# TIGER-AI-Lab/AnyV2V

Measured on AMD Instinct MI355X. Metric: frames/sec for 16fx512x512 DDIM-inversion+PnP-edit; spatial-attn MFMA % of peak, higher is better.
Workload: dtype f16; 1 GPU; BASELINE config 3 per GPU: 1 clip x 16f x 512x512, 50-step DDIM inversion (UNet B=1) + 50-step PnP edit (UNet B=3, cfg 9.0, conv+spatial+temporal injection on every step); a bench step = 1 inversion step + 1 edit step = 1/50 clip; I2VGen-XL 3D-UNet 1.42B params, random init; frames=16, hip_graphs=True, finite=True

## Files before the change

anyv2v_amd/_lib.py:

```python
from __future__ import annotations

import ctypes as C
import os

_HERE = os.path.dirname(os.path.abspath(__file__))
LIB_PATH = os.path.join(_HERE, "libanyv2v_hip.so")
ABI_VERSION = 105


class HipExtensionMissing(RuntimeError):
    pass


class HipKernelError(RuntimeError):
    pass


class GemmDesc(C.Structure):
    _fields_ = [
        ("A0", C.c_void_p), ("A1", C.c_void_p), ("W", C.c_void_p), ("C", C.c_void_p),
        ("bias", C.c_void_p), ("rowvec", C.c_void_p), ("R", C.c_void_p),
        ("M", C.c_int32), ("N", C.c_int32), ("C0", C.c_int32), ("C1", C.c_int32),
        ("lda0", C.c_int32), ("lda1", C.c_int32), ("ldc", C.c_int32), ("ldr", C.c_int32),
        ("ldrv", C.c_int32), ("rowvec_div", C.c_int32), ("mode", C.c_int32),
        ("Hi", C.c_int32), ("Wi", C.c_int32), ("Ho", C.c_int32), ("Wo", C.c_int32),
        ("stride", C.c_int32), ("up", C.c_int32), ("asym", C.c_int32), ("F", C.c_int32), ("HW", C.c_int32),
        ("act", C.c_int32), ("flags", C.c_int32),
        ("workspace", C.c_void_p), ("workspace_bytes", C.c_int64),
        ("ln_c1", C.c_void_p), ("ln_eps", C.c_float), ("reserved0", C.c_int32),
        ("gn_stats", C.c_void_p), ("gn_stats_floats", C.c_int64), ("gn_rows_per_group", C.c_int32), ("gn_groups", C.c_int32),
    ]

ANYV2V_GEMM_NAIVE = 1 << 0
ANYV2V_GEMM_LDS_DMA = 1 << 1
ANYV2V_GEMM_NO_BIG = 1 << 2
ANYV2V_GEMM_FORCE_BIG = 1 << 3
ANYV2V_GEMM_NO_SPLITK = 1 << 4
ANYV2V_GEMM_PROBE_TRACE = 1 << 5
ANYV2V_GEMM_PROBE_KO_SHIFT = 6
ANYV2V_GEMM_NO_WS = 1 << 9
ANYV2V_GEMM_FORCE_WS = 1 << 10
ANYV2V_GEMM_NF4 = 1 << 11
ANYV2V_GEMM_NF5 = 1 << 12
ANYV2V_GEMM_RASTER_SHIFT = 13
ANYV2V_GEMM_RASTER_NFAST = 1 << 16
ANYV2V_GEMM_PP = 1 << 17
ANYV2V_GEMM_NO_PP = 1 << 18
ANYV2V_GEMM_PP_192 = 1 << 19
ANYV2V_GEMM_PP_256 = 1 << 20
ANYV2V_GEMM_SW = 1 << 21
ANYV2V_GEMM_NO_SW = 1 << 22
ANYV2V_GEMM_PROBE_SW_KO_SHIFT = 23
ANYV2V_GEMM_STREAMK = 1 << 26
ANYV2V_GEMM_FORCE_STREAMK = 1 << 27
ANYV2V_GEMM_SWH = 1 << 28
ANYV2V_GEMM_PROBE_KORDER_SHIFT = 29


class FFDesc(C.Structure):
    _fields_ = [
        ("X", C.c_void_p), ("W1", C.c_void_p), ("b1", C.c_void_p), ("W2", C.c_void_p), ("b2", C.c_void_p), ("R", C.c_void_p),
        ("Y", C.c_void_p), ("M", C.c_int32), ("C", C.c_int32), ("H", C.c_int32), ("ldx", C.c_int32), ("ldr", C.c_int32),
        ("ldy", C.c_int32), ("flags", C.c_int32), ("reserved0", C.c_int32),
    ]


class AttnDesc(C.Structure):
    _fields_ = [
        ("Q", C.c_void_p), ("K", C.c_void_p), ("V", C.c_void_p), ("O", C.c_void_p),
        ("ldq", C.c_int32), ("ldk", C.c_int32), ("ldv", C.c_int32), ("ldo", C.c_int32),
        ("batch", C.c_int32), ("heads", C.c_int32), ("Sq", C.c_int32), ("Sk", C.c_int32),
        ("inner", C.c_int32),
        ("q_outer", C.c_int64), ("q_inner", C.c_int64), ("q_seq", C.c_int64),
        ("kv_outer", C.c_int64), ("kv_inner", C.c_int64), ("kv_seq", C.c_int64),
        ("kv_div", C.c_int32), ("qk_mod", C.c_int32), ("scale", C.c_float), ("flags", C.c_int32),
    ]


_VP, _I32, _I64, _F32 = C.c_void_p, C.c_int32, C.c_int64, C.c_float
SYMBOLS = {
    "anyv2v_gemm_f16": (C.c_int, [C.POINTER(GemmDesc), _VP]),
    "anyv2v_gemm_gn_stats_floats": (C.c_int64, [C.POINTER(GemmDesc)]),
    "anyv2v_gemm_gn_launches": (C.c_int64, [_I32]),
    "anyv2v_ff_geglu_f16": (C.c_int, [C.POINTER(FFDesc), _VP]),
    "anyv2v_groupnorm_f16": (C.c_int, [_VP, _VP, _I32, _I32, _VP, _VP, _VP, _VP, _I32, _I32, _I32, _F32, _I32, _VP]),
    "anyv2v_groupnorm_scratch_floats": (C.c_int64, [_I32, _I32, _I32]),
    "anyv2v_groupnorm_stats_floats": (C.c_int64, [_I32, _I32, _I32]),
    "anyv2v_groupnorm_apply_stats_f16": (C.c_int, [_VP, _VP, _VP, _VP, _VP, C.POINTER(C.c_int32), _F32, _I32, _VP]),
    "anyv2v_groupnorm_partial_floats": (C.c_int64, [_I32, _I32, _I32, _I32]),
    "anyv2v_groupnorm_partial_f16": (C.c_int, [_VP, _VP, _I32, _I32, _VP, _I32, _I32, _I32, _VP]),
    "anyv2v_groupnorm_apply_f16": (C.c_int, [_VP, _VP, _I32, _I32, _VP, _VP, _VP, _VP, _I32, _I32, _I32, _F32, _I32, _I32, _VP]),
    "anyv2v_groupnorm_pivot_f16": (C.c_int, [_VP, _VP, _I32, _I32, _VP, _I32, _I32, _I32, _I32, _VP]),
    "anyv2v_groupnorm_partial_pivot_f16": (C.c_int, [_VP, _VP, _I32, _I32, _VP, _VP, _I32, _I32, _I32, _VP]),
    "anyv2v_groupnorm_apply_pivot_f16": (C.c_int, [_VP, _VP, _I32, _I32, _VP, _VP, _VP, _VP, _VP, _I32, _I32, _I32, _F32, _I32, _I32, _VP]),
    "anyv2v_layernorm_f16": (C.c_int, [_VP, _VP, _VP, _VP, _I32, _I32, _F32, _VP]),
    "anyv2v_attention_f16": (C.c_int, [C.POINTER(AttnDesc), _VP]),
    "anyv2v_attention_small_f16": (C.c_int, [C.POINTER(AttnDesc), _I32, _VP]),
    "anyv2v_attention_bias_f16": (C.c_int, [C.POINTER(AttnDesc), _I32, _VP, _VP]),
    "anyv2v_softmax_rows_f32_f16": (C.c_int, [_VP, _I32, _VP, _I32, _I32, _I32, _F32, _VP]),
    "anyv2v_silu_f16": (C.c_int, [_VP, _VP, _I64, _VP]),
    "anyv2v_add_f16": (C.c_int, [_VP, _VP, _VP, _I64, _VP]),
    "anyv2v_timestep_embedding_f16": (C.c_int, [_VP, _VP, _I32, _I32, _VP]),
    "anyv2v_ncfhw_to_tokens_f16": (C.c_int, [_VP, _VP, _I32, _I32, _I32, _I32, _I32, _I32, _VP]),
    "anyv2v_tokens_to_ncfhw_f16": (C.c_int, [_VP, _VP, _I32, _I32, _I32, _I32, _I32, _I32, _VP]),
    "anyv2v_adaptive_avgpool_f16": (C.c_int, [_VP, _VP, _I32, _I32, _I32, _I32, _I32, _I32, _VP]),
    "anyv2v_copy_cols_f16": (C.c_int, [_VP, _I32, _I32, _VP, _I32, _I32, _I64, _I32, _VP]),
    "anyv2v_gather_rows_f16": (C.c_int, [_VP, _I32, _I32, _VP, _VP, _I32, _I32, _I64, _I32, _VP]),
    "anyv2v_freeu_f16": (C.c_int, [_VP, _I32, _VP, _I32, _I32, _F32, _VP, _I32, _VP, _I32, _I32, _F32, _I32, _I32, _I32, _VP]),
    "anyv2v_tile_blend_f16": (C.c_int, [_VP, _I64, _I32, _I32, _VP, _VP, _VP, _VP, _I32, _I32, _VP, _I32, _I32, _I32, _VP]),
    "anyv2v_rotary_f16":(C.c_int, [_VP, _I32, _I64, _I32, _I32, _I32, _I32, _I32, _I32, C.c_float, _VP]),
    "anyv2v_cfg_ddim_step_f16": (C.c_int, [_VP, _I32, _I32, _I32, _F32, _VP, _VP, _VP, _I32, _I32, _I32, _VP]),
    "anyv2v_ddim_step_f16": (C.c_int, [_VP, _VP, _VP, _F32, _F32, _F32, _F32, _I64, _VP]),
    "anyv2v_guided_step_f16": (C.c_int, [_VP, _I64, _I32, _I32, _I32, _F32, _F32, _I32, _F32, _F32, _F32, _F32, _VP, _VP, _VP]),
    "anyv2v_guided_step_noise_f16": (C.c_int, [_VP, _I64, _I32, _I32, _I32, _F32, _F32, _I32, _F32, _F32, _F32, _F32, _VP, _VP, _VP, _F32, _VP]),
    "anyv2v_set_batch_hint": (C.c_int, [_I32, _I32]),
    "anyv2v_last_error": (C.c_char_p, []),
    "anyv2v_version": (C.c_int, []),
    "anyv2v_selftest": (C.c_int, [_VP, _I64, _VP]),
}

_lib = None


def load():
    global _lib
    if _lib is not None:
        return _lib
    if not os.path.isfile(LIB_PATH):
        raise HipExtensionMissing(
            f"{LIB_PATH} not found: the HIP kernels are the product path and there is no fallback. "
            f"Build with `make -C {os.path.join(_HERE, 'csrc')}` (or `python -c 'import __graft_entry__ as g; g.build()'`).")
    lib = C.CDLL(LIB_PATH)
    for name, (res, args) in SYMBOLS.items():
        fn = getattr(lib, name)
        fn.restype = res
        fn.argtypes = args
    if lib.anyv2v_version() < ABI_VERSION:
        raise HipExtensionMissing(f"{LIB_PATH} is ABI {lib.anyv2v_version()}, this binding needs >= {ABI_VERSION}: rebuild it "
                                  f"(`make -C {os.path.join(_HERE, 'csrc')}`)")
    _lib = lib
    return lib


def check(rc: int, what: str = ""):
    if rc != 0:
        msg = load().anyv2v_last_error()
        raise HipKernelError(f"{what} failed (rc={rc}): {msg.decode() if msg else ''}")
```

anyv2v_amd/ops.py:

```python
from __future__ import annotations

import ctypes as C
import os
from typing import Optional

import torch

from . import _lib
from ._lib import AttnDesc, GemmDesc

MODE_LINEAR, MODE_CONV2D, MODE_TEMPORAL = 0, 1, 2
ACT_NONE, ACT_SILU, ACT_GELU, ACT_GEGLU, ACT_F32OUT = 0, 1, 2, 3, 4

FORCE_NAIVE = False
ATTN_FLAGS = int(os.environ.get("ANYV2V_ATTN_FLAGS", "0"))
GEMM_FLAGS = int(os.environ.get("ANYV2V_GEMM_FLAGS", "0"))
USE_GLDS = os.environ.get("ANYV2V_GLDS", "1") == "1"


def _parse_switch(value: Optional[str]) -> bool:
    return (value or "0").strip() == "1"


GN_EPILOGUE = _parse_switch(os.environ.get("ANYV2V_GN_EPILOGUE"))
# ... 92 lines not shown
               | GEMM_FLAGS)
    if ln is not None:
        c1, eps = ln
        assert c1.dtype == torch.float32 and c1.is_cuda and c1.numel() >= N and c1.is_contiguous()
        d.ln_c1, d.ln_eps = _p(c1), float(eps)
    ws = _workspace(a0.device)
    d.workspace, d.workspace_bytes = ws.data_ptr(), ws.numel() * 4
    if gn is not None:
        stats, rows_per_group, groups = gn
        d.gn_rows_per_group, d.gn_groups = int(rows_per_group), int(groups)
        if stats is not None:
            assert stats.dtype == torch.float32 and stats.is_cuda and stats.is_contiguous()
            d.gn_stats, d.gn_stats_floats = stats.data_ptr(), stats.numel()
    if _query:
        return int(lib.anyv2v_gemm_gn_stats_floats(C.byref(d)))
    _lib.check(lib.anyv2v_gemm_f16(C.byref(d), _stream()), "anyv2v_gemm_f16")
    return out


def gemm_gn_stats_floats(a0: torch.Tensor, w: torch.Tensor, *, rows_per_group: int, groups: int = 32, **kw) -> int:
    return gemm(a0, w, gn=(None, rows_per_group, groups), _query=True, **kw)


def gn_launches(reset: bool = True) -> int:
    return int(_lib.load().anyv2v_gemm_gn_launches(int(reset)))


def gn_stats_floats(M: int, rows_per_group: int, groups: int = 32) -> int:
    return int(_lib.load().anyv2v_groupnorm_stats_floats(int(M), int(rows_per_group), int(groups)))


def groupnorm_from_stats(x: torch.Tensor, gamma, beta, stats: torch.Tensor, rows_per_group: int, *, groups: int = 32,
                         eps: float = 1e-5, silu: bool = False, out=None):
    lib = _lib.load()
    _rowmajor(x, "X")
    assert x.is_contiguous()
    M, Cc = x.shape
    if out is None:
        out = torch.empty((M, Cc), dtype=torch.float16, device=x.device)
    assert out.is_contiguous()
    assert stats.dtype == torch.float32 and stats.is_contiguous() and stats.numel() >= gn_stats_floats(M, rows_per_group, groups) > 0
    sizes = (C.c_int32 * 5)(M, Cc, rows_per_group, groups, min(stats.numel(), 2 ** 31 - 1))
    _lib.check(lib.anyv2v_groupnorm_apply_stats_f16(_p(x), _p(out), _p(gamma), _p(beta), _p(stats), sizes, eps, int(silu),
                                                    _stream()), "anyv2v_groupnorm_apply_stats_f16")
    return out


FF_FUSED = os.environ.get("ANYV2V_FF_FUSED", "1") == "1"


def ff_fused_supported(M: int, C: int, H: int) -> bool:
    return FF_FUSED and not FORCE_NAIVE and USE_GLDS and C == 320 and H == 1280 and M * _HINT[0] // _HINT[1] >= 32768


def ff_pack_w2(w2: torch.Tensor) -> torch.Tensor:
    C, H = w2.shape
    assert H % 32 == 0
    q, e = torch.arange(4).view(4, 1), torch.arange(8).view(1, 8)
    perm = torch.where(e < 4, 4 * q + e, 16 + 4 * q + (e - 4)).reshape(32).to(w2.device)
    return w2.view(C, H // 32, 32)[:, :, perm].permute(1, 0, 2).contiguous()


def ff_geglu(x: torch.Tensor, w1p: torch.Tensor, b1p: torch.Tensor, w2s: torch.Tensor, b2: torch.Tensor, residual=None, out=None):
    lib = _lib.load()
    M, Cc = x.shape
    H = w2s.shape[0] * 32
    assert x.dtype == torch.float16 and x.stride(1) == 1 and w1p.is_contiguous() and w2s.is_contiguous()
    assert tuple(w1p.shape) == (2 * H, Cc) and tuple(w2s.shape) == (H // 32, Cc, 32) and b1p.numel() == 2 * H and b2.numel() == Cc
    if out is None:
        out = torch.empty((M, Cc), dtype=torch.float16, device=x.device)
    for name, t in (("residual", residual), ("out", out)):
        assert t is None or (tuple(t.shape) == (M, Cc) and t.dtype == torch.float16 and t.stride(1) == 1 and t.device == x.device), \
            f"ff_geglu: {name} must be an fp16 [{M}, {Cc}] matrix with unit column stride on {x.device}"
    d = _lib.FFDesc()
    d.X, d.W1, d.b1, d.W2, d.b2, d.Y = _p(x), _p(w1p), _p(b1p), _p(w2s), _p(b2), _p(out)
    d.R = _p(residual) if residual is not None else None
    d.M, d.C, d.H = M, Cc, H
    d.ldx, d.ldy, d.ldr = x.stride(0), out.stride(0), (residual.stride(0) if residual is not None else 0)
    d.flags = d.reserved0 = 0
    _lib.check(lib.anyv2v_ff_geglu_f16(C.byref(d), _stream()), "anyv2v_ff_geglu_f16")
    return out


def ln_gemm_supported(M: int, K: int, N: int, act: int = ACT_NONE, hinted: bool = True) -> bool:
    if FORCE_NAIVE or not USE_GLDS or (GEMM_FLAGS & (_lib.ANYV2V_GEMM_NO_WS | _lib.ANYV2V_GEMM_NO_BIG)) or (M * _HINT[0] // _HINT[1] if hinted else M) < 32768:
        return False
    if K == 320:
        return N % 160 == 0 and N // 160 <= 32
    return K == 512 and act == ACT_GEGLU and N % 128 == 0 and N // 128 <= 32


def ln_fold(w: torch.Tensor, bias: Optional[torch.Tensor], gamma: torch.Tensor, beta: torch.Tensor):
    wf = w.float() * gamma.float()[None, :]
    w16 = wf.to(torch.float16).contiguous()
    c1 = w16.float().sum(1).contiguous()
    b = w.float() @ beta.float()
    if bias is not None:
        b = b + bias.float()
    return w16, b.to(torch.float16).contiguous(), c1


def gn_scratch_floats(M: int, rows_per_group: int, groups: int = 32) -> int:
    return (M // rows_per_group) * groups * 2 * 257


def groupnorm(x0: torch.Tensor, gamma, beta, stats: torch.Tensor, rows_per_group: int, *, x1=None, groups: int = 32,
              eps: float = 1e-5, silu: bool = False, out=None, shard=None):
    if shard is not None:
        return _groupnorm_sharded(x0, gamma, beta, stats, rows_per_group, x1, groups, eps, silu, out, shard)
    lib = _lib.load()
    _rowmajor(x0, "X0")
    assert x0.is_contiguous()
    M, C0 = x0.shape
    C1 = 0
    if x1 is not None:
        _rowmajor(x1, "X1")
        assert x1.is_contiguous() and x1.shape[0] == M
        C1 = x1.shape[1]
    if out is None:
        out = torch.empty((M, C0 + C1), dtype=torch.float16, device=x0.device)
    assert out.is_contiguous()
    need = gn_scratch_floats(M, rows_per_group, groups)
    assert stats.dtype == torch.float32 and stats.numel() >= need, "GroupNorm scratch too small"
    _lib.check(lib.anyv2v_groupnorm_f16(_p(x0), _p(x1), C0, C1, _p(out), _p(gamma), _p(beta), _p(stats), M,
                                        rows_per_group, groups, eps, int(silu), _stream()), "anyv2v_groupnorm_f16")
    return out


def _groupnorm_sharded(x0, gamma, beta, stats, rows_per_group, x1, groups, eps, silu, out, shard):
    lib = _lib.load()
    shards, all_reduce_sum = shard
    _rowmajor(x0, "X0")
    assert x0.is_contiguous()
    M, C0 = x0.shape
    C1 = 0
    if x1 is not None:
        _rowmajor(x1, "X1")
        assert x1.is_contiguous() and x1.shape[0] == M
        C1 = x1.shape[1]
    if out is None:
        out = torch.empty((M, C0 + C1), dtype=torch.float16, device=x0.device)
    assert out.is_contiguous()
    n = int(lib.anyv2v_groupnorm_partial_floats(M, rows_per_group, groups, C0 + C1))
    npiv = (M // rows_per_group) * groups
    assert n > 0 and stats.dtype == torch.float32 and stats.numel() >= n + npiv, "GroupNorm scratch too small"
    piv = stats[n:n + npiv]
    _lib.check(lib.anyv2v_groupnorm_pivot_f16(_p(x0), _p(x1), C0, C1, _p(piv), M, rows_per_group, groups, int(shards), _stream()),
               "anyv2v_groupnorm_pivot_f16")
    all_reduce_sum(piv)
    _lib.check(lib.anyv2v_groupnorm_partial_pivot_f16(_p(x0), _p(x1), C0, C1, _p(piv), _p(stats), M, rows_per_group, groups,
                                                      _stream()), "anyv2v_groupnorm_partial_pivot_f16")
    all_reduce_sum(stats[:n])
    _lib.check(lib.anyv2v_groupnorm_apply_pivot_f16(_p(x0), _p(x1), C0, C1, _p(out), _p(gamma), _p(beta), _p(piv), _p(stats), M,
                                                    rows_per_group, groups, eps, int(silu), int(shards), _stream()),
               "anyv2v_groupnorm_apply_pivot_f16")
    return out


def layernorm(x: torch.Tensor, gamma, beta, eps: float = 1e-5, out=None):
    lib = _lib.load()
    _rowmajor(x, "X")
    assert x.is_contiguous()
    M, Cc = x.shape
    if out is None:
        out = torch.empty_like(x)
    _lib.check(lib.anyv2v_layernorm_f16(_p(x), _p(out), _p(gamma), _p(beta), M, Cc, eps, _stream()), "anyv2v_layernorm_f16")
# ... 234 lines not shown
```

anyv2v_amd/unet.py:

```python
from __future__ import annotations

import copy
import math
import os

from dataclasses import dataclass
from typing import List, Optional, Tuple

import torch
import torch.nn as nn

from . import ops
from .ops import ACT_GEGLU, ACT_GELU, ACT_NONE, ACT_SILU, MODE_CONV2D, MODE_TEMPORAL


@dataclass
class I2VGenXLUNetConfig:
    in_channels: int = 4
    out_channels: int = 4
    block_out_channels: Tuple[int, ...] = (320, 640, 1280, 1280)
    layers_per_block: int = 2
    norm_num_groups: int = 32
    cross_attention_dim: int = 1024
    attention_head_dim: int = 64
# ... 293 lines not shown
        out = proc(self, hs, encoder_hidden_states=ehs)
        if geom.kind != "spatial":
            out = out.view(geom.B, geom.HW, geom.F, C).permute(0, 2, 1, 3)
        out = out.reshape(-1, C).contiguous()
        return ops.add(out, residual)


class GEGLU(nn.Module):
    def __init__(self, dim_in, dim_out):
        super().__init__()
        self.proj = Linear(dim_in, dim_out * 2)
        self.dim_out = dim_out
        self._w = self._b = None

    def pack(self):
        w, b = self.proj.weight.data, self.proj.bias.data
        n = self.dim_out
        assert n % 16 == 0
        wh, wg = w[:n].view(n // 16, 16, -1), w[n:].view(n // 16, 16, -1)
        self._w = torch.stack([wh, wg], 1).reshape(2 * n, -1).contiguous()
        bh, bg = b[:n].view(n // 16, 16), b[n:].view(n // 16, 16)
        self._b = torch.stack([bh, bg], 1).reshape(2 * n).contiguous()


class GELUProj(nn.Module):
    def __init__(self, dim_in, dim_out):
        super().__init__()
        self.proj = Linear(dim_in, dim_out)


class FeedForward(nn.Module):
    def __init__(self, dim, inner_dim=None, activation_fn="geglu"):
        super().__init__()
        inner_dim = inner_dim or dim * 4
        self.geglu = activation_fn == "geglu"
        act = GEGLU(dim, inner_dim) if self.geglu else GELUProj(dim, inner_dim)
        self.net = nn.ModuleList([act, Identity(), Linear(inner_dim, dim)])

    def pack(self):
        lin = self.net[2]
        self._w2s = ops.ff_pack_w2(lin.weight.data) if (self.geglu and tuple(lin.weight.shape) == (320, 1280)) else None

    def run(self, h, residual, ln_in=None):
        w2s = getattr(self, "_w2s", None)
        if ln_in is None and w2s is not None and ops.ff_fused_supported(h.shape[0], h.shape[1], w2s.shape[0] * 32):
            return ops.ff_geglu(h, self.net[0]._w, self.net[0]._b, w2s, self.net[2].bias, residual=residual)
        if ln_in is not None:
            x, (w_in, b_in, c1_in), ln_eps = ln_in
            g = ops.gemm(x, w_in, bias=b_in, act=ACT_GEGLU, ln=(c1_in, ln_eps))
        elif self.geglu:
            g = ops.gemm(h, self.net[0]._w, bias=self.net[0]._b, act=ACT_GEGLU)
        else:
            g = ops.gemm(h, self.net[0].proj.weight, bias=self.net[0].proj.bias, act=ACT_GELU)
        return ops.gemm(g, self.net[2].weight, bias=self.net[2].bias, residual=residual)


class BasicTransformerBlock(nn.Module):
    def __init__(self, dim, heads, dim_head, cross_attention_dim=None, double_self_attention=False):
        super().__init__()
        self.norm1 = LayerNorm(dim)
        self.attn1 = Attention(dim, None, heads, dim_head)
        self.norm2 = LayerNorm(dim)
        self.attn2 = Attention(dim, None if double_self_attention else cross_attention_dim, heads, dim_head)
        self.norm3 = LayerNorm(dim)
        self.ff = FeedForward(dim)

    def pack(self):
        self._ln = {}
        dim = self.norm1.weight.shape[0]
        if dim not in (320, 512) or _NO_LN_FOLD:
            return
        cat = lambda a: torch.cat([a.to_q.weight.data, a.to_k.weight.data, a.to_v.weight.data], 0)
        if dim == 320:
            self._ln["attn1"] = ops.ln_fold(cat(self.attn1), None, self.norm1.weight.data, self.norm1.bias.data)
            w2 = self.attn2.to_q.weight.data if self.attn2.is_cross else cat(self.attn2)
            self._ln["attn2"] = ops.ln_fold(w2, None, self.norm2.weight.data, self.norm2.bias.data)
        if self.ff.geglu and _LN_FOLD_FF:
            g = self.ff.net[0]
            w, b, c1 = ops.ln_fold(g.proj.weight.data, g.proj.bias.data, self.norm3.weight.data, self.norm3.bias.data)
            n = g.dim_out
            il = lambda t: torch.stack([t[:n].reshape(n // 16, 16, *t.shape[1:]), t[n:].reshape(n // 16, 16, *t.shape[1:])], 1) \
                .reshape(2 * n, *t.shape[1:]).contiguous()
            self._ln["ff"] = (il(w), il(b), il(c1))

    def _fold(self, name, proc_ok, M, N, act=ACT_NONE, per_branch=False):
        f = getattr(self, "_ln", {}).get(name)
        return f if (f is not None and proc_ok and ops.ln_gemm_supported(M, self.norm1.weight.shape[0], N, act, hinted=not per_branch)) else None

    def run(self, ctx, x, geom: Geom, expand=None, shrink=None):
        dim = x.shape[1]
        rows_b = lambda t, g: t.shape[0] // g.B
        f = self._fold("attn1", isinstance(self.attn1.processor, HipAttnProcessor), rows_b(x, geom), 3 * dim, per_branch=True)
        if f is not None:
            x = self.attn1.run(ctx, None, geom, residual=x, ln_in=(x, f, self.norm1.eps))
        else:
            h = ops.layernorm(x, self.norm1.weight, self.norm1.bias, self.norm1.eps)
            x = self.attn1.run(ctx, h, geom, residual=x)
        if expand is not None:
            after = getattr(ctx, "batch_hint_after", None)
            ctx, geom = expand
            x = expand_shared(x, ctx)
            if after is not None:
                ops.set_batch_hint(*after)
        if shrink is not None:
            x = x[x.shape[0] // 3:]
            geom = shrink
            ops.set_batch_hint(3, 2)
        kv = ctx.kv_for(self.attn2) if self.attn2.is_cross else None
        f = self._fold("attn2", isinstance(self.attn2.processor, HipAttnProcessor), rows_b(x, geom), dim if self.attn2.is_cross else 3 * dim,
                       per_branch=True)
        if f is not None:
            x = self.attn2.run(ctx, None, geom, residual=x, kv=kv, ln_in=(x, f, self.norm2.eps))
        else:
            h = ops.layernorm(x, self.norm2.weight, self.norm2.bias, self.norm2.eps)
            x = self.attn2.run(ctx, h, geom, residual=x, kv=kv)
        f = self._fold("ff", True, x.shape[0], 8 * dim, ACT_GEGLU)
        if f is not None:
            return self.ff.run(None, residual=x, ln_in=(x, f, self.norm3.eps))
        h = ops.layernorm(x, self.norm3.weight, self.norm3.bias, self.norm3.eps)
        return self.ff.run(h, residual=x)


class Transformer2DModel(nn.Module):
    def __init__(self, heads, dim_head, in_channels, cross_attention_dim, groups):
        super().__init__()
        inner = heads * dim_head
        self.norm = GroupNorm(groups, in_channels, eps=1e-6)
        self.proj_in = Linear(in_channels, inner)
        self.transformer_blocks = nn.ModuleList([BasicTransformerBlock(inner, heads, dim_head, cross_attention_dim)])
        self.proj_out = Linear(inner, in_channels)

    def run(self, ctx, x, H, W, full_ctx=None):
        HW = H * W
        h = ops.groupnorm(x, self.norm.weight, self.norm.bias, ctx.stats, HW, groups=self.norm.num_groups,
                          eps=self.norm.eps)
        h = ops.gemm(h, self.proj_in.weight, bias=self.proj_in.bias)
        geom = Geom("spatial", ctx.B, ctx.F, HW)
        for i, blk in enumerate(self.transformer_blocks):
            if full_ctx is not None and i == 0:
                h = blk.run(ctx, h, geom, expand=(full_ctx, Geom("spatial", full_ctx.B, full_ctx.F, HW)))
                ctx, geom = full_ctx, Geom("spatial", full_ctx.B, full_ctx.F, HW)
                x = expand_shared(x, full_ctx)
            else:
                h = blk.run(ctx, h, geom)
        return ops.gemm(h, self.proj_out.weight, bias=self.proj_out.bias, residual=x)


class TransformerTemporalModel(nn.Module):
    def __init__(self, heads, dim_head, in_channels, groups):
        super().__init__()
        inner = heads * dim_head
        self.norm = GroupNorm(groups, in_channels, eps=1e-6)
        self.proj_in = Linear(in_channels, inner)
        self.transformer_blocks = nn.ModuleList(
            [BasicTransformerBlock(inner, heads, dim_head, None, double_self_attention=True)])
        self.proj_out = Linear(inner, in_channels)

    def run(self, ctx, x, H, W):
        fp = getattr(ctx, "fp", None)
        return self._run(ctx, x, H * W, None) if fp is None else fp.temporal(ctx, x, H * W, self._run)

    def _run(self, ctx, x, HW, shard):
        h = ops.groupnorm(x, self.norm.weight, self.norm.bias, ctx.stats, ctx.F * HW, groups=self.norm.num_groups,
                          eps=self.norm.eps, shard=shard)
        h = ops.gemm(h, self.proj_in.weight, bias=self.proj_in.bias)
        geom = Geom("temporal", ctx.B, ctx.F, HW)
        drop = shard is None and getattr(ctx, "drop_tail_at", None) is self and not self.transformer_blocks[0].attn2.is_cross
        for i, blk in enumerate(self.transformer_blocks):
            if drop and i == 0:
                h = blk.run(ctx, h, geom, shrink=Geom("temporal", ctx.B - 1, ctx.F, HW))
                geom = Geom("temporal", ctx.B - 1, ctx.F, HW)
                x = x[x.shape[0] // 3:]
            else:
                h = blk.run(ctx, h, geom)
        return ops.gemm(h, self.proj_out.weight, bias=self.proj_out.bias, residual=x)


class Upsample2D(nn.Module):
    def __init__(self, channels):
        super().__init__()
        self.conv = Conv2d(channels, channels, 3, padding=1)


class Downsample2D(nn.Module):
    def __init__(self, channels):
        super().__init__()
        self.conv = Conv2d(channels, channels, 3, stride=2, padding=1)


class ResnetBlock2D(nn.Module):

    def __init__(self, in_channels, out_channels, temb_channels, groups, eps=1e-5):
        super().__init__()
        self.in_channels, self.out_channels = in_channels, out_channels
# ... 540 lines not shown
```

include/anyv2v_hip.h:

```cpp
#ifndef ANYV2V_HIP_H
#define ANYV2V_HIP_H

#include <stdint.h>

#ifdef __cplusplus
extern "C" {
#endif

#define ANYV2V_OK 0
#define ANYV2V_EINVAL (-1)
#define ANYV2V_EUNSUPPORTED (-2)

#define ANYV2V_GEMM_NAIVE (1 << 0)
#define ANYV2V_GEMM_LDS_DMA (1 << 1)
#define ANYV2V_GEMM_NO_BIG (1 << 2)
#define ANYV2V_GEMM_FORCE_BIG (1 << 3)
#define ANYV2V_GEMM_NO_SPLITK (1 << 4)
#define ANYV2V_GEMM_PROBE_TRACE (1 << 5)
#define ANYV2V_GEMM_PROBE_KO_SHIFT 6
#define ANYV2V_GEMM_NO_WS (1 << 9)
#define ANYV2V_GEMM_FORCE_WS (1 << 10)
#define ANYV2V_GEMM_NF4 (1 << 11)
#define ANYV2V_GEMM_NF5 (1 << 12)
#define ANYV2V_GEMM_RASTER_SHIFT 13
#define ANYV2V_GEMM_RASTER_NFAST (1 << 16)
#define ANYV2V_GEMM_PP (1 << 17)
#define ANYV2V_GEMM_NO_PP (1 << 18)
#define ANYV2V_GEMM_PP_192 (1 << 19)
#define ANYV2V_GEMM_PP_256 (1 << 20)
#define ANYV2V_GEMM_SW (1 << 21)
#define ANYV2V_GEMM_NO_SW (1 << 22)
#define ANYV2V_GEMM_PROBE_SW_KO_SHIFT 23
#define ANYV2V_GEMM_STREAMK (1 << 26)
#define ANYV2V_GEMM_FORCE_STREAMK (1 << 27)
#define ANYV2V_GEMM_SWH (1 << 28)
#define ANYV2V_GEMM_PROBE_KORDER_SHIFT 29
typedef struct AnyV2VGemmDesc {
    const void* A0;
    const void* A1;
    const void* W;
    void* C;
    const void* bias;
    const void* rowvec;
    const void* R;
    int32_t M, N;
    int32_t C0, C1;
    int32_t lda0, lda1, ldc, ldr, ldrv, rowvec_div;
    int32_t mode;
    int32_t Hi, Wi, Ho, Wo, stride, up;
    int32_t asym;
    int32_t F, HW;
    int32_t act;
    int32_t flags;
    void* workspace;
    int64_t workspace_bytes;
    const float* ln_c1;
    float ln_eps;
    int32_t reserved0;
    float* gn_stats;
    int64_t gn_stats_floats;
    int32_t gn_rows_per_group;
    int32_t gn_groups;
} AnyV2VGemmDesc;

int anyv2v_gemm_f16(const AnyV2VGemmDesc* d, void* stream);
int64_t anyv2v_gemm_gn_stats_floats(const AnyV2VGemmDesc* d);
int64_t anyv2v_gemm_gn_launches(int32_t reset);

typedef struct AnyV2VFFDesc {
    const void* X;
    const void* W1;
    const void* b1;
    const void* W2;
    const void* b2;
    const void* R;
    void* Y;
    int32_t M, C, H;
    int32_t ldx, ldr, ldy;
    int32_t flags;
    int32_t reserved0;
} AnyV2VFFDesc;

int anyv2v_ff_geglu_f16(const AnyV2VFFDesc* d, void* stream);

int64_t anyv2v_groupnorm_scratch_floats(int32_t M, int32_t rows_per_group, int32_t G);
int anyv2v_groupnorm_f16(const void* X0, const void* X1, int32_t C0, int32_t C1, void* Y, const void* gamma,
                         const void* beta, float* stats, int32_t M, int32_t rows_per_group, int32_t G, float eps,
                         int32_t silu, void* stream);
int64_t anyv2v_groupnorm_stats_floats(int32_t M, int32_t rows_per_group, int32_t G);
int anyv2v_groupnorm_apply_stats_f16(const void* X, void* Y, const void* gamma, const void* beta, float* stats,
                                     const int32_t* sizes, float eps, int32_t silu, void* stream);

int64_t anyv2v_groupnorm_partial_floats(int32_t M, int32_t rows_per_group, int32_t G, int32_t C);
int anyv2v_groupnorm_pivot_f16(const void* X0, const void* X1, int32_t C0, int32_t C1, float* pivot, int32_t M,
                               int32_t rows_per_group, int32_t G, int32_t shards, void* stream);
int anyv2v_groupnorm_partial_pivot_f16(const void* X0, const void* X1, int32_t C0, int32_t C1, const float* pivot,
                                       float* stats, int32_t M, int32_t rows_per_group, int32_t G, void* stream);
int anyv2v_groupnorm_apply_pivot_f16(const void* X0, const void* X1, int32_t C0, int32_t C1, void* Y, const void* gamma,
                                     const void* beta, const float* pivot, const float* stats, int32_t M,
                                     int32_t rows_per_group, int32_t G, float eps, int32_t silu, int32_t shards, void* stream);
int anyv2v_groupnorm_partial_f16(const void* X0, const void* X1, int32_t C0, int32_t C1, float* stats, int32_t M,
                                 int32_t rows_per_group, int32_t G, void* stream);
int anyv2v_groupnorm_apply_f16(const void* X0, const void* X1, int32_t C0, int32_t C1, void* Y, const void* gamma,
                               const void* beta, const float* stats, int32_t M, int32_t rows_per_group, int32_t G,
                               float eps, int32_t silu, int32_t shards, void* stream);

int anyv2v_layernorm_f16(const void* X, void* Y, const void* gamma, const void* beta, int32_t M, int32_t C,
                         float eps, void* stream);

typedef struct AnyV2VAttnDesc {
    const void* Q;
    const void* K;
    const void* V;
    void* O;
    int32_t ldq, ldk, ldv, ldo;
    int32_t batch, heads, Sq, Sk;
    int32_t inner;
    int64_t q_outer, q_inner, q_seq;
    int64_t kv_outer, kv_inner, kv_seq;
    int32_t kv_div;
    int32_t qk_mod;
    float scale;
    int32_t flags;
} AnyV2VAttnDesc;

int anyv2v_attention_f16(const AnyV2VAttnDesc* d, void* stream);

int anyv2v_attention_small_f16(const AnyV2VAttnDesc* d, int32_t head_dim, void* stream);
int anyv2v_attention_bias_f16(const AnyV2VAttnDesc* d, int32_t head_dim, const float* bias, void* stream);

int anyv2v_silu_f16(const void* X, void* Y, int64_t n, void* stream);
int anyv2v_add_f16(const void* A, const void* B, void* Y, int64_t n, void* stream);
int anyv2v_timestep_embedding_f16(const float* t, void* out, int32_t B, int32_t dim, void* stream);
int anyv2v_ncfhw_to_tokens_f16(const void* X, void* Y, int32_t B, int32_t C, int32_t F, int32_t HW, int32_t ldy,
                               int32_t col0, void* stream);
int anyv2v_tokens_to_ncfhw_f16(const void* X, void* Y, int32_t B, int32_t C, int32_t F, int32_t HW, int32_t ldx,
                               int32_t col0, void* stream);
int anyv2v_adaptive_avgpool_f16(const void* X, void* Y, int32_t N, int32_t Hi, int32_t Wi, int32_t Ho, int32_t Wo,
                                int32_t C, void* stream);
int anyv2v_gather_rows_f16(const void* X, int32_t ldx, int32_t xcol0, const int32_t* idx, void* Y, int32_t ldy, int32_t ycol0,
                           int64_t M, int32_t C, void* stream);
int anyv2v_rotary_f16(void* X, int32_t ld, int64_t rows, int32_t col0, int32_t rot_dim, int32_t n_windows, int32_t window_stride,
                      int32_t rows_per_pos, int32_t n_pos, float theta, void* stream);
int anyv2v_copy_cols_f16(const void* X, int32_t ldx, int32_t xcol0, void* Y, int32_t ldy, int32_t ycol0, int64_t M,
                         int32_t C, void* stream);

int anyv2v_freeu_f16(const void* hidden, int32_t ld_hidden, void* hidden_out, int32_t ld_hidden_out, int32_t C_hidden, float b,
                     const void* skip, int32_t ld_skip, void* skip_out, int32_t ld_skip_out, int32_t C_skip, float s,
                     int32_t n_img, int32_t H, int32_t W, void* stream);

int anyv2v_tile_blend_f16(const void* tiles, int64_t tile_rows, int32_t ld, int32_t C, const int32_t* plan_host,
                          const double* weight_host, const int32_t* plan_dev, const double* weight_dev, int32_t nty, int32_t ntx,
                          void* out, int32_t n_img, int32_t H, int32_t W, void* stream);

int anyv2v_softmax_rows_f32_f16(const float* S, int32_t lds, void* P, int32_t ldp, int32_t rows, int32_t cols, float scale,
                                void* stream);

int anyv2v_cfg_ddim_step_f16(const void* Vtok, int32_t ldv, int32_t b_unc, int32_t b_cond, float guidance,
                             const float* coef, const void* lat, void* out, int32_t C, int32_t F, int32_t HW,
                             void* stream);

int anyv2v_ddim_step_f16(const void* V, const void* X, void* Y, float sa_t, float sb_t, float sa_p, float sb_p,
                         int64_t n, void* stream);

int anyv2v_guided_step_f16(const void* E, int64_t n, int32_t b_unc, int32_t b_img, int32_t b_txt, float g_img, float g_txt,
                           int32_t prediction, float sa_t, float sb_t, float sa_p, float sb_p, const void* X, void* Y, void* stream);
// ... 16 lines not shown
```

Measured before the change: 3.037 frames/s.

## Fuse LayerNorm, QKV, temporal attention and out-projection for C=320 blocks

Adds a single HIP kernel for the C=320, 5-head, F=16 temporal self-attention blocks. It performs the folded LayerNorm, QKV projection, per-pixel 16-frame softmax attention, output projection, bias and residual add in one pass. Pre-packed, swizzled weights are streamed into LDS with double-buffered DMA. This removes the intermediate QKV and attention-output round trips through global memory and the several launches the separate path used. The fused path is skipped when PnP injection is active, so on the edit pass it only runs on steps without injection, and it is hard-coded to one shape.

```diff
diff --git a/anyv2v_amd/_lib.py b/anyv2v_amd/_lib.py
--- a/anyv2v_amd/_lib.py
+++ b/anyv2v_amd/_lib.py
@@ -65,6 +65,14 @@
     ]
 
 
+class TAttnDesc(C.Structure):
+    _fields_ = [
+        ("X", C.c_void_p), ("WP", C.c_void_p), ("AUX", C.c_void_p), ("Y", C.c_void_p),
+        ("batch", C.c_int32), ("F", C.c_int32), ("HW", C.c_int32), ("C", C.c_int32), ("heads", C.c_int32),
+        ("ldx", C.c_int32), ("ldy", C.c_int32), ("scale", C.c_float), ("eps", C.c_float), ("flags", C.c_int32),
+    ]
+
+
 class AttnDesc(C.Structure):
     _fields_ = [
         ("Q", C.c_void_p), ("K", C.c_void_p), ("V", C.c_void_p), ("O", C.c_void_p),
@@ -83,6 +91,7 @@
     "anyv2v_gemm_gn_stats_floats": (C.c_int64, [C.POINTER(GemmDesc)]),
     "anyv2v_gemm_gn_launches": (C.c_int64, [_I32]),
     "anyv2v_ff_geglu_f16": (C.c_int, [C.POINTER(FFDesc), _VP]),
+    "anyv2v_temporal_attn_c320_f16": (C.c_int, [C.POINTER(TAttnDesc), _VP]),
     "anyv2v_groupnorm_f16": (C.c_int, [_VP, _VP, _I32, _I32, _VP, _VP, _VP, _VP, _I32, _I32, _I32, _F32, _I32, _VP]),
     "anyv2v_groupnorm_scratch_floats": (C.c_int64, [_I32, _I32, _I32]),
     "anyv2v_groupnorm_stats_floats": (C.c_int64, [_I32, _I32, _I32]),
diff --git a/anyv2v_amd/csrc/tattn_fused.hip b/anyv2v_amd/csrc/tattn_fused.hip
--- /dev/null
+++ b/anyv2v_amd/csrc/tattn_fused.hip
@@ -0,0 +1,292 @@
+#include "gemm_common.h"
+
+namespace {
+constexpr int TA_C = 320, TA_F = 16, TA_HEADS = 5;
+constexpr int TA_STAGE = 24 * 1024;
+constexpr int TA_NSTEP = 7;
+constexpr int TA_QLD = 144;
+constexpr int TA_MAT = 16 * TA_QLD, TA_SEQ = 3 * TA_MAT, TA_PAIR = 2 * TA_SEQ;
+constexpr int TA_LDS = 2 * TA_STAGE + 4 * TA_PAIR;
+constexpr int TA_AUX_B = 3 * TA_C, TA_AUX_BO = 6 * TA_C;
+
+struct TAK {
+    const half_t* X;
+    const half_t* WP;
+    const float* AUX;
+    half_t* Y;
+    int ldx, ldy, HW, nseq, nstrips;
+    float eps, scale_log2;
+};
+
+typedef __fp16 ta_fp16x4 __attribute__((__vector_size__(8)));
+template <int OFF>
+__device__ __forceinline__ ta_fp16x4 ta_tr16(unsigned addr) {
+    ta_fp16x4 r;
+    asm volatile("ds_read_b64_tr_b16 %0, %1 offset:%2" : "=v"(r) : "v"(addr), "i"(OFF) : "memory");
+    return r;
+}
+__device__ __forceinline__ void ta_w64(unsigned addr, h4 v) { asm volatile("ds_write_b64 %0, %1" ::"v"(addr), "v"(v) : "memory"); }
+#define TA_LGKM(n) do { __builtin_amdgcn_sched_barrier(0); asm volatile("s_waitcnt lgkmcnt(" #n ")" ::: "memory"); __builtin_amdgcn_sched_barrier(0); } while (0)
+#define TA_LGKM_TAIL(left) do { if ((left) >= 2) TA_LGKM(2); else if ((left) == 1) TA_LGKM(1); else TA_LGKM(0); } while (0)
+}
+
+template <int KO = 0>
+__global__ __launch_bounds__(512) void tattn_fused_c320_kernel(const TAK p) {
+    __shared__ __attribute__((aligned(16))) char smem[TA_LDS];
+    const unsigned lds0 = (unsigned)(size_t)(__attribute__((address_space(3))) char*)smem;
+    constexpr unsigned QB = 2 * TA_STAGE;
+
+    const int tid = threadIdx.x, lane = tid & 63;
+    const int w = __builtin_amdgcn_readfirstlane(tid >> 6);
+    const int l15 = lane & 15, lq = lane >> 4;
+    const int half_ = w & 1, pr = w >> 1;
+    const int G = gridDim.x;
+
+    auto dma = [&](int stage, int buf) {
+        const char* src = (const char*)p.WP + (size_t)stage * TA_STAGE + (3 * w) * 1024 + lane * 16;
+#pragma unroll
+        for (int q = 0; q < 3; ++q) glds16((const half_t*)(src + q * 1024), smem + buf * TA_STAGE + (3 * w + q) * 1024);
+    };
+    auto step_sync = [&]() {
+        __builtin_amdgcn_sched_barrier(0);
+        __builtin_amdgcn_s_waitcnt(0x0070);
+        __builtin_amdgcn_s_barrier();
+        __builtin_amdgcn_sched_barrier(0);
+    };
+
+    if (KO != 1) dma(0, 0);
+    step_sync();
+
+    const int rounds = (p.nstrips - (int)blockIdx.x * 4 + G * 4 - 1) / (G * 4);
+    int gs = 0;
+    for (int rd = 0; rd < rounds; ++rd) {
+        const int strip = (rd * G + blockIdx.x) * 4 + pr;
+        const bool live = strip < p.nstrips;
+        const int strip_c = live ? strip : p.nstrips - 1;
+        long long xrow[2];
+        h8 xf[2][10];
+        float mean[2], rstd[2];
+#pragma unroll
+        for (int rf = 0; rf < 2; ++rf) {
+            int s = strip_c * 2 + rf;
+            s = s < p.nseq ? s : p.nseq - 1;
+            const int b = s / p.HW, px = s - b * p.HW;
+            xrow[rf] = ((long long)b * TA_F + l15) * p.HW + px;
+            const half_t* xp = p.X + xrow[rf] * p.ldx + lq * 8;
+#pragma unroll
+            for (int ks = 0; ks < 10; ++ks) xf[rf][ks] = *(const h8*)(xp + ks * 32);
+        }
+#pragma unroll
+        for (int rf = 0; rf < 2; ++rf) {
+            float s = 0.f;
+#pragma unroll
+            for (int ks = 0; ks < 10; ++ks)
+#pragma unroll
+                for (int e = 0; e < 8; ++e) s += (float)xf[rf][ks][e];
+            s += __shfl_xor(s, 16, 64);
+            s += __shfl_xor(s, 32, 64);
+            const float mu = s * (1.0f / TA_C);
+            float d = 0.f;
+#pragma unroll
+            for (int ks = 0; ks < 10; ++ks)
+#pragma unroll
+                for (int e = 0; e < 8; ++e) {
+                    const float c = (float)xf[rf][ks][e] - mu;
+                    d = fmaf(c, c, d);
+                }
+            d += __shfl_xor(d, 16, 64);
+            d += __shfl_xor(d, 32, 64);
+            mean[rf] = mu;
+            rstd[rf] = __builtin_amdgcn_rsqf(d * (1.0f / TA_C) + p.eps);
+        }
+        f4 yacc[20];
+#pragma unroll
+        for (int nf = 0; nf < 20; ++nf) yacc[nf] = (f4){0.f, 0.f, 0.f, 0.f};
+
+        for (int h = 0; h < TA_HEADS; ++h) {
+            f4 acc[2][6];
+            h8 ob[2];
+#pragma unroll
+            for (int s = 0; s < TA_NSTEP; ++s) {
+                const bool last = h == TA_HEADS - 1 && s == TA_NSTEP - 1;
+                if (KO != 1 && (!last || rd + 1 < rounds)) dma(last ? 0 : h * TA_NSTEP + s + 1, (gs + 1) & 1);
+                __builtin_amdgcn_sched_barrier(0);
+                int lane_j = lane;
+                asm volatile("" : "+v"(lane_j));
+                const int l15_ = lane_j & 15, lq_ = lane_j >> 4;
+                const unsigned wb = lds0 + (gs & 1) * TA_STAGE;
+                const unsigned sw0 = ((lq_ ^ (l15_ & 7)) << 4), sw1 = (((4 + lq_) ^ (l15_ & 7)) << 4);
+                const unsigned pairb = lds0 + QB + pr * TA_PAIR;
+                if (s < 5) {
+                    if (s == 0) {
+#pragma unroll
+                        for (int rf = 0; rf < 2; ++rf)
+#pragma unroll
+                            for (int c = 0; c < 6; ++c) acc[rf][c] = (f4){0.f, 0.f, 0.f, 0.f};
+                    }
+                    const unsigned rb = wb + (96 * half_ + l15_) * 128;
+                    const unsigned a0 = rb + sw0, a1 = rb + sw1;
+                    h8 wf[3];
+#define TA_RD_A(I) wf[(I) % 3] = lds_frag((I) >= 6 ? a1 : a0, ((I) % 6) * 2048)
+                    TA_RD_A(0);
+                    TA_RD_A(1);
+                    __builtin_amdgcn_s_setprio(1);
+#pragma unroll
+                    for (int i = 0; i < 12; ++i) {
+                        if (i + 2 < 12) TA_RD_A(i + 2);
+                        TA_LGKM_TAIL(11 - i);
+                        const int ks = 2 * s + i / 6, c = i % 6;
+                        if constexpr (KO == 4) {
+                            asm volatile("" ::"v"(wf[i % 3]), "v"(xf[0][ks]), "v"(xf[1][ks]));
+                        } else {
+                            acc[0][c] = __builtin_amdgcn_mfma_f32_16x16x32_f16(wf[i % 3], xf[0][ks], acc[0][c], 0, 0, 0);
+                            acc[1][c] = __builtin_amdgcn_mfma_f32_16x16x32_f16(wf[i % 3], xf[1][ks], acc[1][c], 0, 0, 0);
+                        }
+                        __builtin_amdgcn_sched_barrier(0);
+                    }
+#undef TA_RD_A
+                    __builtin_amdgcn_s_setprio(0);
+                    if (s == 4) {
+#pragma unroll
+                        for (int c = 0; c < 6; ++c) {
+                            const int colb = 96 * half_ + 16 * c;
+                            const float* ax = p.AUX + h * 192 + colb + 4 * lq_;
+                            const f4 c1 = *(const f4*)ax, bb = *(const f4*)(ax + TA_AUX_B);
+                            const unsigned dst = pairb + (colb >> 6) * TA_MAT + l15_ * TA_QLD + ((colb & 63) + 4 * lq_) * 2;
+#pragma unroll
+                            for (int rf = 0; rf < 2; ++rf) {
+                                h4 o;
+#pragma unroll
+                                for (int r = 0; r < 4; ++r) o[r] = (half_t)fmaf(fmaf(-mean[rf], c1[r], acc[rf][c][r]), rstd[rf], bb[r]);
+                                ta_w64(dst + rf * TA_SEQ, o);
+                            }
+                        }
+                    }
+                } else {
+                    if (s == 5) {
+                        const unsigned ab = pairb + half_ * TA_SEQ;
+                        const unsigned qa = ab + l15_ * TA_QLD + lq_ * 16;
+                        h8 qf[2], kf[2];
+                        qf[0] = lds_frag(qa, 0);
+                        qf[1] = lds_frag(qa, 64);
+                        kf[0] = lds_frag(qa, TA_MAT);
+                        kf[1] = lds_frag(qa, TA_MAT + 64);
+                        const unsigned va = ab + 2 * TA_MAT + (4 * lq_ + (l15_ >> 2)) * TA_QLD + (l15_ & 3) * 8;
+                        ta_fp16x4 vt[4];
+                        vt[0] = ta_tr16<0>(va);
+                        vt[1] = ta_tr16<32>(va);
+                        vt[2] = ta_tr16<64>(va);
+                        vt[3] = ta_tr16<96>(va);
+                        TA_LGKM(0);
+                        if constexpr (KO == 2) {
+                            ob[0] = qf[0];
+                            ob[1] = qf[1];
+                            asm volatile("" ::"v"(kf[0]), "v"(kf[1]), "v"(vt[0]), "v"(vt[1]), "v"(vt[2]), "v"(vt[3]));
+                        } else {
+                            f4 sc = {0.f, 0.f, 0.f, 0.f};
+                            sc = __builtin_amdgcn_mfma_f32_16x16x32_f16(kf[0], qf[0], sc, 0, 0, 0);
+                            sc = __builtin_amdgcn_mfma_f32_16x16x32_f16(kf[1], qf[1], sc, 0, 0, 0);
+                            float mx = fmaxf(fmaxf(sc[0], sc[1]), fmaxf(sc[2], sc[3]));
+                            mx = fmaxf(mx, __shfl_xor(mx, 16, 64));
+                            mx = fmaxf(mx, __shfl_xor(mx, 32, 64));
+                            float sum = 0.f;
+                            h4 pf;
+#pragma unroll
+                            for (int r = 0; r < 4; ++r) {
+                                const float e = exp2f((sc[r] - mx) * p.scale_log2);
+                                sum += e;
+                                pf[r] = (half_t)e;
+                            }
+                            sum += __shfl_xor(sum, 16, 64);
+                            sum += __shfl_xor(sum, 32, 64);
+                            const float inv = 1.0f / sum;
+#pragma unroll
+                            for (int db = 0; db < 4; ++db) {
+                                h4 vf;
+#pragma unroll
+                                for (int j = 0; j < 4; ++j) vf[j] = (half_t)vt[db][j];
+                                f4 o = {0.f, 0.f, 0.f, 0.f};
+                                o = __builtin_amdgcn_mfma_f32_16x16x16f16(vf, pf, o, 0, 0, 0);
+#pragma unroll
+                                for (int r = 0; r < 4; ++r) ob[db >> 1][4 * (db & 1) + r] = (half_t)(o[r] * inv);
+                            }
+                        }
+                    }
+                    const unsigned rb = wb + l15_ * 128;
+                    const unsigned a0 = rb + sw0, a1 = rb + sw1;
+                    h8 wf[3];
+#define TA_RD_C(J) wf[(J) % 3] = lds_frag(((J) & 1) ? a1 : a0, ((J) >> 1) * 2048)
+                    TA_RD_C(0);
+                    TA_RD_C(1);
+                    __builtin_amdgcn_s_setprio(1);
+#pragma unroll
+                    for (int j = 0; j < 20; ++j) {
+                        if (j + 2 < 20) TA_RD_C(j + 2);
+                        TA_LGKM_TAIL(19 - j);
+                        const int nf = 10 * (s - 5) + (j >> 1);
+                        if constexpr (KO == 3)
+                            asm volatile("" ::"v"(wf[j % 3]), "v"(ob[j & 1]));
+                        else
+                            yacc[nf] = __builtin_amdgcn_mfma_f32_16x16x32_f16(wf[j % 3], ob[j & 1], yacc[nf], 0, 0, 0);
+                        __builtin_amdgcn_sched_barrier(0);
+                    }
+#undef TA_RD_C
+                    __builtin_amdgcn_s_setprio(0);
+                }
+                step_sync();
+                ++gs;
+            }
+        }
+
+        const int sq = strip * 2 + half_;
+        if (live && sq < p.nseq) {
+            half_t* yp = p.Y + (half_ ? xrow[1] : xrow[0]) * p.ldy + lq * 8;
+            const float* bo = p.AUX + TA_AUX_BO + lq * 8;
+#pragma unroll
+            for (int m = 0; m < 10; ++m) {
+                const h8 xr = half_ ? xf[1][m] : xf[0][m];
+                const f4 b0 = *(const f4*)(bo + 32 * m), b1 = *(const f4*)(bo + 32 * m + 4);
+                h8 o;
+#pragma unroll
+                for (int r = 0; r < 4; ++r) {
+                    o[r] = (half_t)(yacc[2 * m][r] + b0[r] + (float)xr[r]);
+                    o[4 + r] = (half_t)(yacc[2 * m + 1][r] + b1[r] + (float)xr[4 + r]);
+                }
+                *(h8*)(yp + 32 * m) = o;
+            }
+        }
+    }
+}
+
+extern "C" int anyv2v_temporal_attn_c320_f16(const AnyV2VTAttnDesc* d, void* stream) {
+    AV_CHECK(d != nullptr, "temporal_attn: null descriptor");
+    AV_CHECK(d->X && d->WP && d->AUX && d->Y, "temporal_attn: null X / WP / AUX / Y");
+    if (d->C != TA_C || d->heads * 64 != d->C || d->F != TA_F) {
+        anyv2v_set_error("temporal_attn: only C = 320, 5 heads x 64, F = 16 is implemented (got C %d, heads %d, F %d)", d->C, d->heads, d->F);
+        return ANYV2V_EUNSUPPORTED;
+    }
+    AV_CHECK(d->batch > 0 && d->HW > 0, "temporal_attn: bad batch %d / HW %d", d->batch, d->HW);
+    AV_CHECK((long long)d->batch * d->HW * TA_F < (1ll << 31), "temporal_attn: %lld rows do not fit 31 bits", (long long)d->batch * d->HW * TA_F);
+    AV_CHECK(d->ldx >= TA_C && d->ldy >= TA_C && d->ldx % 8 == 0 && d->ldy % 8 == 0, "temporal_attn: ldx, ldy must be >= 320 and multiples of 8");
+    AV_CHECK(av_aligned16(d->X) && av_aligned16(d->WP) && av_aligned16(d->AUX) && av_aligned16(d->Y),
+             "temporal_attn: X / WP / AUX / Y must be 16-byte aligned");
+    TAK k;
+    k.X = (const half_t*)d->X; k.WP = (const half_t*)d->WP; k.AUX = (const float*)d->AUX; k.Y = (half_t*)d->Y;
+    k.ldx = d->ldx; k.ldy = d->ldy; k.HW = d->HW;
+    k.nseq = d->batch * d->HW;
+    k.nstrips = (k.nseq + 1) / 2;
+    k.eps = d->eps;
+    k.scale_log2 = d->scale * 1.4426950408889634f;
+    const int blocks = (k.nstrips + 3) / 4;
+    const dim3 grid(blocks < 256 ? blocks : 256);
+#ifdef ANYV2V_EXPERIMENTS
+    switch (d->flags & 7) {
+#define AV_TA_KO(n) case n: hipLaunchKernelGGL((tattn_fused_c320_kernel<n>), grid, dim3(512), 0, (hipStream_t)stream, k); return av_launch_status("tattn_fused<KO>");
+        AV_TA_KO(1) AV_TA_KO(2) AV_TA_KO(3) AV_TA_KO(4)
+#undef AV_TA_KO
+        default: break;
+    }
+#endif
+    hipLaunchKernelGGL(tattn_fused_c320_kernel<0>, grid, dim3(512), 0, (hipStream_t)stream, k);
+    return av_launch_status("tattn_fused_c320");
+}
diff --git a/anyv2v_amd/ops.py b/anyv2v_amd/ops.py
--- a/anyv2v_amd/ops.py
+++ b/anyv2v_amd/ops.py
@@ -198,6 +198,56 @@
     return out
 
 
+TATTN_FUSED = os.environ.get("ANYV2V_TATTN_FUSED", "1") == "1"
+
+
+def temporal_attn_supported(rows_per_branch: int, C: int, heads: int, F: int) -> bool:
+    return (TATTN_FUSED and not FORCE_NAIVE and USE_GLDS and C == 320 and heads * 64 == C and F == 16
+            and rows_per_branch >= 32768 and rows_per_branch % F == 0)
+
+
+def tattn_pack(ln_fold_, w_o: torch.Tensor, b_o: torch.Tensor, heads: int = 5):
+    w, b, c1 = ln_fold_
+    Cc = w.shape[1]
+    assert tuple(w.shape) == (3 * Cc, Cc) and Cc == heads * 64 == 320 and tuple(w_o.shape) == (Cc, Cc) and b_o.numel() == Cc
+    dev = w.device
+    ar = lambda n: torch.arange(n, device=dev)
+    a = w.view(3, heads, 64, Cc // 64, 64).permute(1, 3, 0, 2, 4).reshape(heads, Cc // 64, 192, 64)
+    nf, q, r = ar(20).view(20, 1, 1), ar(4).view(1, 4, 1), ar(4).view(1, 1, 4)
+    n_of_row = (32 * (nf // 2) + 8 * q + 4 * (nf % 2) + r).reshape(Cc)
+    ks, e = ar(2).view(2, 1, 1), ar(8).view(1, 1, 8)
+    d_of_col = (32 * ks + 16 * (e // 4) + 4 * q + e % 4).reshape(64)
+    c = w_o.view(Cc, heads, 64)[n_of_row][:, :, d_of_col].permute(1, 0, 2).reshape(heads, 2, 160, 64)
+    c = torch.cat([c, torch.zeros((heads, 2, 32, 64), dtype=c.dtype, device=dev)], 2)
+    st = torch.cat([a, c], 1).reshape(heads, 7, 192, 8, 8)
+    src_chunk = ar(8).view(1, 8) ^ (ar(192).view(192, 1) & 7)
+    wp = st[:, :, ar(192).view(192, 1), src_chunk].reshape(heads, 7, 192, 64).to(torch.float16).contiguous()
+    order = lambda t: t.float().view(3, heads, 64).permute(1, 0, 2).reshape(3 * Cc)
+    aux = torch.cat([order(c1), order(b), b_o.float().reshape(Cc)]).contiguous()
+    return wp, aux
+
+
+def temporal_attn_c320(x: torch.Tensor, wp: torch.Tensor, aux: torch.Tensor, *, batch: int, F: int, HW: int, scale: float,
+                       eps: float, heads: int = 5, out=None):
+    lib = _lib.load()
+    _rowmajor(x, "X")
+    M, Cc = x.shape
+    assert M == batch * F * HW, f"temporal_attn: {M} rows are not batch {batch} x F {F} x HW {HW}"
+    assert wp.dtype == torch.float16 and wp.is_contiguous() and tuple(wp.shape) == (heads, 7, 192, 64)
+    assert aux.dtype == torch.float32 and aux.is_contiguous() and aux.numel() == 7 * Cc
+    if out is None:
+        out = torch.empty((M, Cc), dtype=torch.float16, device=x.device)
+    _rowmajor(out, "Y")
+    assert tuple(out.shape) == (M, Cc) and out.device == x.device
+    d = _lib.TAttnDesc()
+    d.X, d.WP, d.AUX, d.Y = _p(x), _p(wp), _p(aux), _p(out)
+    d.batch, d.F, d.HW, d.C, d.heads = batch, F, HW, Cc, heads
+    d.ldx, d.ldy = x.stride(0), out.stride(0)
+    d.scale, d.eps, d.flags = scale, eps, 0
+    _lib.check(lib.anyv2v_temporal_attn_c320_f16(C.byref(d), _stream()), "anyv2v_temporal_attn_c320_f16")
+    return out
+
+
 def ln_gemm_supported(M: int, K: int, N: int, act: int = ACT_NONE, hinted: bool = True) -> bool:
     if FORCE_NAIVE or not USE_GLDS or (GEMM_FLAGS & (_lib.ANYV2V_GEMM_NO_WS | _lib.ANYV2V_GEMM_NO_BIG)) or (M * _HINT[0] // _HINT[1] if hinted else M) < 32768:
         return False
diff --git a/anyv2v_amd/unet.py b/anyv2v_amd/unet.py
--- a/anyv2v_amd/unet.py
+++ b/anyv2v_amd/unet.py
@@ -399,6 +399,18 @@
             il = lambda t: torch.stack([t[:n].reshape(n // 16, 16, *t.shape[1:]), t[n:].reshape(n // 16, 16, *t.shape[1:])], 1) \
                 .reshape(2 * n, *t.shape[1:]).contiguous()
             self._ln["ff"] = (il(w), il(b), il(c1))
+        self._tattn = {}
+        if dim == 320 and not self.attn2.is_cross and self.attn1.heads == 5:
+            for name, a in (("attn1", self.attn1), ("attn2", self.attn2)):
+                self._tattn[name] = ops.tattn_pack(self._ln[name], a.to_out[0].weight.data, a.to_out[0].bias.data, a.heads)
+
+    def _tattn_fused(self, name, attn, ctx, geom, rows_b):
+        t = getattr(self, "_tattn", {}).get(name)
+        proc = attn.processor
+        if (t is None or geom.kind != "temporal" or not isinstance(proc, HipAttnProcessor) or pnp_on(proc.t, proc.injection_schedule)
+                or getattr(ctx, "fp", None) is not None or not ops.temporal_attn_supported(rows_b, attn.inner_dim, attn.heads, geom.F)):
+            return None
+        return t
 
     def _fold(self, name, proc_ok, M, N, act=ACT_NONE, per_branch=False):
         f = getattr(self, "_ln", {}).get(name)
@@ -408,7 +420,10 @@
         dim = x.shape[1]
         rows_b = lambda t, g: t.shape[0] // g.B
         f = self._fold("attn1", isinstance(self.attn1.processor, HipAttnProcessor), rows_b(x, geom), 3 * dim, per_branch=True)
-        if f is not None:
+        tf = self._tattn_fused("attn1", self.attn1, ctx, geom, rows_b(x, geom)) if f is not None else None
+        if tf is not None:
+            x = ops.temporal_attn_c320(x, *tf, batch=geom.B, F=geom.F, HW=geom.HW, scale=self.attn1.scale, eps=self.norm1.eps)
+        elif f is not None:
             x = self.attn1.run(ctx, None, geom, residual=x, ln_in=(x, f, self.norm1.eps))
         else:
             h = ops.layernorm(x, self.norm1.weight, self.norm1.bias, self.norm1.eps)
@@ -426,7 +441,10 @@
         kv = ctx.kv_for(self.attn2) if self.attn2.is_cross else None
         f = self._fold("attn2", isinstance(self.attn2.processor, HipAttnProcessor), rows_b(x, geom), dim if self.attn2.is_cross else 3 * dim,
                        per_branch=True)
-        if f is not None:
+        tf = self._tattn_fused("attn2", self.attn2, ctx, geom, rows_b(x, geom)) if (f is not None and kv is None) else None
+        if tf is not None:
+            x = ops.temporal_attn_c320(x, *tf, batch=geom.B, F=geom.F, HW=geom.HW, scale=self.attn2.scale, eps=self.norm2.eps)
+        elif f is not None:
             x = self.attn2.run(ctx, None, geom, residual=x, kv=kv, ln_in=(x, f, self.norm2.eps))
         else:
             h = ops.layernorm(x, self.norm2.weight, self.norm2.bias, self.norm2.eps)
diff --git a/include/anyv2v_hip.h b/include/anyv2v_hip.h
--- a/include/anyv2v_hip.h
+++ b/include/anyv2v_hip.h
@@ -82,6 +82,19 @@
 } AnyV2VFFDesc;
 
 int anyv2v_ff_geglu_f16(const AnyV2VFFDesc* d, void* stream);
+
+typedef struct AnyV2VTAttnDesc {
+    const void* X;
+    const void* WP;
+    const void* AUX;
+    void* Y;
+    int32_t batch, F, HW, C, heads;
+    int32_t ldx, ldy;
+    float scale, eps;
+    int32_t flags;
+} AnyV2VTAttnDesc;
+
+int anyv2v_temporal_attn_c320_f16(const AnyV2VTAttnDesc* d, void* stream);
 
 int64_t anyv2v_groupnorm_scratch_floats(int32_t M, int32_t rows_per_group, int32_t G);
 int anyv2v_groupnorm_f16(const void* X0, const void* X1, int32_t C0, int32_t C1, void* Y, const void* gamma,
```

Measured after the change: 3.064 frames/s (median of 6 runs). About the same (+0.9%).
